# UbiquityRobotics/fiducials

Measured on AMD Instinct MI355X. Metric: frames/sec @1920x1080 20-marker (aruco detect + pose hot path), higher is better.
Workload: dtype u8

## Files before the change

fiducials_amd/csrc/fid_kernels.hip:

```cpp
#include <hip/hip_runtime.h>
#include <stdint.h>
#include <float.h>
#include <limits.h>

#include <type_traits>
#include <utility>

#include "fid_device.h"
#include "../../include/fid_abi.h"

#define WAVE 64

__device__ __forceinline__ int lane_id() { return threadIdx.x & (WAVE - 1); }

__device__ __forceinline__ unsigned long long ballot64(int pred) { return __ballot(pred); }

#define FID_DPP(OLD, V, CTRL, RMASK) __builtin_amdgcn_update_dpp((OLD), (V), (CTRL), (RMASK), 0xf, false)
#define FID_DPP_SCAN_STEPS(STEP) STEP(0x111, 0xf) STEP(0x112, 0xf) STEP(0x114, 0xf) STEP(0x118, 0xf) STEP(0x142, 0xa) STEP(0x143, 0xc)

__device__ __forceinline__ int wave_iscan(int v)
{
#define S_(C, M) v += FID_DPP(0, v, C, M);
    FID_DPP_SCAN_STEPS(S_)
#undef S_
    return v;
}

__device__ __forceinline__ unsigned long long wave_max_u64(unsigned long long k)
{
    unsigned lo = (unsigned)k, hi = (unsigned)(k >> 32);
#define S_(C, M)                                                                      \
    {                                                                                 \
        const unsigned ol = (unsigned)FID_DPP(0, (int)lo, C, M), oh = (unsigned)FID_DPP(0, (int)hi, C, M); \
        const bool gt = oh > hi || (oh == hi && ol > lo);                             \
        lo = gt ? ol : lo;                                                            \
        hi = gt ? oh : hi;                                                            \
    }
    FID_DPP_SCAN_STEPS(S_)
#undef S_
    lo = (unsigned)__builtin_amdgcn_readlane((int)lo, 63);
    hi = (unsigned)__builtin_amdgcn_readlane((int)hi, 63);
    return ((unsigned long long)hi << 32) | lo;
}

__device__ __forceinline__ void wave_argmax_first(unsigned d, unsigned idx, unsigned &md, unsigned &mi)
{
    unsigned v = d;
#define S_(C, M)                                                  \
    {                                                             \
        const unsigned o = (unsigned)FID_DPP(0, (int)v, C, M);    \
        v = o > v ? o : v;                                        \
    }
    FID_DPP_SCAN_STEPS(S_)
#undef S_
    md = (unsigned)__builtin_amdgcn_readlane((int)v, 63);
    unsigned w = d == md ? idx : 0xffffffffu;
#define S_(C, M)                                                  \
    {                                                             \
        const unsigned o = (unsigned)FID_DPP(-1, (int)w, C, M);   \
        w = o < w ? o : w;                                        \
    }
    FID_DPP_SCAN_STEPS(S_)
#undef S_
    mi = (unsigned)__builtin_amdgcn_readlane((int)w, 63);
}

__device__ __forceinline__ double wave_max_nonneg_f64(double v)
{
    unsigned long long u = __double_as_longlong(v);
    unsigned lo = (unsigned)u, hi = (unsigned)(u >> 32);
#define S_(C, M)                                                                                           \
    {                                                                                                      \
        const unsigned ol = (unsigned)FID_DPP(0, (int)lo, C, M), oh = (unsigned)FID_DPP(0, (int)hi, C, M); \
        const bool gt = oh > hi || (oh == hi && ol > lo);  \
        lo = gt ? ol : lo;                                                                                 \
        hi = gt ? oh : hi;                                                                                 \
    }
    FID_DPP_SCAN_STEPS(S_)
#undef S_
    lo = (unsigned)__builtin_amdgcn_readlane((int)lo, 63);
    hi = (unsigned)__builtin_amdgcn_readlane((int)hi, 63);
    return __longlong_as_double(((unsigned long long)hi << 32) | lo);
}

__device__ __forceinline__ int wave_min_i32(int v)
{
#define S_(C, M)                                  \
    {                                             \
        const int o = FID_DPP(INT_MAX, v, C, M);  \
        v = o < v ? o : v;                        \
    }
    FID_DPP_SCAN_STEPS(S_)
#undef S_
    return __builtin_amdgcn_readlane(v, 63);
}
__device__ __forceinline__ int wave_min_i32_dpp(int v) { return wave_min_i32(v); }

__device__ __forceinline__ int wave_sum_i32(int v) { return __builtin_amdgcn_readlane(wave_iscan(v), 63); }

__device__ __forceinline__ long long wave_sum_i64(long long v)
{
    unsigned lo = (unsigned)v, hi = (unsigned)((unsigned long long)v >> 32);
#define S_(C, M)                                                                      \
    {                                                                                 \
        const unsigned ol = (unsigned)FID_DPP(0, (int)lo, C, M), oh = (unsigned)FID_DPP(0, (int)hi, C, M); \
        const unsigned long long t = (((unsigned long long)hi << 32) | lo) + (((unsigned long long)oh << 32) | ol); \
        lo = (unsigned)t;                                                             \
        hi = (unsigned)(t >> 32);                                                     \
    }
    FID_DPP_SCAN_STEPS(S_)
#undef S_
    lo = (unsigned)__builtin_amdgcn_readlane((int)lo, 63);
    hi = (unsigned)__builtin_amdgcn_readlane((int)hi, 63);
    return (long long)(((unsigned long long)hi << 32) | lo);
}

__device__ __forceinline__ double bcast_f64(double v, int src)
{
    const unsigned long long u = __double_as_longlong(v);
    const int l = __builtin_amdgcn_readfirstlane(src);
    const unsigned lo = (unsigned)__builtin_amdgcn_readlane((int)(unsigned)u, l);
    const unsigned hi = (unsigned)__builtin_amdgcn_readlane((int)(unsigned)(u >> 32), l);
    return __longlong_as_double(((unsigned long long)hi << 32) | lo);
}

__device__ __forceinline__ double shfl_f64(double v, int src)
{
    unsigned long long u = __double_as_longlong(v);
    unsigned lo = __shfl((unsigned)u, src, WAVE);
    unsigned hi = __shfl((unsigned)(u >> 32), src, WAVE);
    return __longlong_as_double(((unsigned long long)hi << 32) | lo);
}

__global__ __launch_bounds__(256) void k_to_gray(const uint8_t *__restrict__ src, int stride, long long fstride,
                                                  int enc, uint8_t *__restrict__ dst, int W, int H, int F)
{
    long long total = (long long)W * H * F;
    for (long long i = (long long)blockIdx.x * blockDim.x + threadIdx.x; i < total; i += (long long)gridDim.x * blockDim.x) {
        int x = (int)(i % W);
        long long t = i / W;
        int y = (int)(t % H);
        int f = (int)(t / H);
        const uint8_t *s = src + f * fstride + (long long)y * stride;
        uint8_t v;
        if (enc == FID_ENC_MONO8) {
            v = s[x];
        } else {
            const int px = (enc == FID_ENC_BGRA8 || enc == FID_ENC_RGBA8) ? 4 : 3;
            int c0 = s[px * x], c1 = s[px * x + 1], c2 = s[px * x + 2];
            const bool bfirst = enc == FID_ENC_BGR8 || enc == FID_ENC_BGRA8;
            int b = bfirst ? c0 : c2, r = bfirst ? c2 : c0;
            v = (uint8_t)((b * 3735 + c1 * 19235 + r * 9798 + (1 << 14)) >> 15);
        }
        dst[i] = v;
    }
}

__device__ __forceinline__ int k0_gray(int b, int g, int r) { return (b * 3735 + g * 19235 + r * 9798 + (1 << 14)) >> 15; }
__device__ __forceinline__ int k0_scale16(const uint8_t *p, bool be)
{
    const unsigned v = be ? ((unsigned)p[0] << 8) | p[1] : (unsigned)p[0] | ((unsigned)p[1] << 8);
    const float a = (float)(255. / 65535.);
    const int r = __float2int_rn((float)v * a);
    return r < 0 ? 0 : (r > 255 ? 255 : r);
}
__device__ __forceinline__ int k0_sat8(int v) { return v < 0 ? 0 : (v > 255 ? 255 : v); }
__device__ __forceinline__ int k0_bayer_gray(const int n[9], bool is_green, int hv)
{
    int own, other, green;
    if (is_green) {
        green = n[4];
        other = (n[1] + n[7] + 1) >> 1;
        own = (n[3] + n[5] + 1) >> 1;
    } else {
        own = n[4];
        green = (n[1] + n[3] + n[5] + n[7] + 2) >> 2;
        other = (n[0] + n[2] + n[6] + n[8] + 2) >> 2;
    }
    const int b = hv > 0 ? other : own, r = hv > 0 ? own : other;
    return k0_gray(b, green, r);
}
__global__ __launch_bounds__(256) void k_raw_to_gray(const uint8_t *__restrict__ src, int stride, long long fstride, int enc,
                                                      uint8_t *__restrict__ dst, int W, int H)
{
    const int x0 = ((int)blockIdx.x * 64 + (int)threadIdx.x) * 4, y = (int)blockIdx.y * 4 + (int)threadIdx.y, f = blockIdx.z;
    if (x0 >= W || y >= H) return;
    const uint8_t *img = src + (long long)f * fstride;
    uint8_t *o = dst + ((long long)f * H + y) * W + x0;
    const int n = W - x0 < 4 ? W - x0 : 4;
    const int base = enc & 0xff;
    const bool be = (enc & FID_ENC_BIGENDIAN) != 0;
    int g[4] = {0, 0, 0, 0};
    if (base >= FID_ENC_BAYER_RGGB8 && base <= FID_ENC_BAYER_GRBG8) {
        const int blue0 = (base == FID_ENC_BAYER_RGGB8 || base == FID_ENC_BAYER_GRBG8) ? -1 : 1;
        const int green0 = (base == FID_ENC_BAYER_GBRG8 || base == FID_ENC_BAYER_GRBG8) ? 1 : 0;
        const int yy = y < 1 ? 1 : (y > H - 2 ? H - 2 : y);
        const int hv = ((yy - 1) & 1) ? -blue0 : blue0;
        const int gs = green0 ^ ((yy - 1) & 1);
        const uint8_t *r0 = img + (long long)(yy - 1) * stride, *r1 = r0 + stride, *r2 = r1 + stride;
        if (x0 >= 1 && x0 + 4 <= W - 1) {
            int a0[6], a1[6], a2[6];
#pragma unroll
            for (int k = 0; k < 6; k++) {
                a0[k] = r0[x0 - 1 + k];
                a1[k] = r1[x0 - 1 + k];
                a2[k] = r2[x0 - 1 + k];
            }
#pragma unroll
            for (int k = 0; k < 4; k++) {
                const int nb[9] = {a0[k], a0[k + 1], a0[k + 2], a1[k], a1[k + 1], a1[k + 2], a2[k], a2[k + 1], a2[k + 2]};
                g[k] = k0_bayer_gray(nb, (gs ^ ((x0 + k - 1) & 1)) != 0, hv);
            }
        } else {
            for (int k = 0; k < n; k++) {
                const int x = x0 + k, xx = x < 1 ? 1 : (x > W - 2 ? W - 2 : x);
                const int nb[9] = {r0[xx - 1], r0[xx], r0[xx + 1], r1[xx - 1], r1[xx], r1[xx + 1], r2[xx - 1], r2[xx], r2[xx + 1]};
                g[k] = k0_bayer_gray(nb, (gs ^ ((xx - 1) & 1)) != 0, hv);
            }
        }
    } else if (base == FID_ENC_MONO16) {
        const uint8_t *s = img + (long long)y * stride + 2 * x0;
        for (int k = 0; k < n; k++) g[k] = k0_scale16(s + 2 * k, be);
    } else if (base >= FID_ENC_BGR16 && base <= FID_ENC_RGBA16) {
        const int ch = (base == FID_ENC_BGRA16 || base == FID_ENC_RGBA16) ? 4 : 3;
        const bool bfirst = base == FID_ENC_BGR16 || base == FID_ENC_BGRA16;
        const uint8_t *s = img + (long long)y * stride + 2 * ch * x0;
        for (int k = 0; k < n; k++) {
            const int c0 = k0_scale16(s + 2 * (ch * k), be), c1 = k0_scale16(s + 2 * (ch * k + 1), be), c2 = k0_scale16(s + 2 * (ch * k + 2), be);
            g[k] = k0_gray(bfirst ? c0 : c2, c1, bfirst ? c2 : c0);
        }
    } else {
        const int CY = 1220542, CUB = 2116026, CUG = -409993, CVG = -852492, CVR = 1673527, SH = 20;
        const uint8_t *s = img + (long long)y * stride + 2 * x0;
        for (int k = 0; k < n; k += 2) {
            const int u = s[2 * k] - 128, y0 = s[2 * k + 1], v = s[2 * k + 2] - 128, y1 = s[2 * k + 3];
            const int ruv = (1 << (SH - 1)) + CVR * v, guv = (1 << (SH - 1)) + CVG * v + CUG * u, buv = (1 << (SH - 1)) + CUB * u;
            const int p0 = (y0 - 16 > 0 ? y0 - 16 : 0) * CY, p1 = (y1 - 16 > 0 ? y1 - 16 : 0) * CY;
            g[k] = k0_gray(k0_sat8((p0 + buv) >> SH), k0_sat8((p0 + guv) >> SH), k0_sat8((p0 + ruv) >> SH));
            g[k + 1] = k0_gray(k0_sat8((p1 + buv) >> SH), k0_sat8((p1 + guv) >> SH), k0_sat8((p1 + ruv) >> SH));
        }
    }
    if (n == 4 && (((unsigned long long)o) & 3ull) == 0) {
        *reinterpret_cast<unsigned *>(o) = (unsigned)g[0] | ((unsigned)g[1] << 8) | ((unsigned)g[2] << 16) | ((unsigned)g[3] << 24);
    } else {
        for (int k = 0; k < n; k++) o[k] = (uint8_t)g[k];
    }
}

template <int TX, int TY, int NT>
__global__ __launch_bounds__(NT) void k_threshold(const uint8_t *__restrict__ gray, long long gfstride,
                                                   uint32_t *__restrict__ masks, const DevParams P)
{
    extern __shared__ uint32_t I[];
    const int R = P.rmax;
    const int RW = TX + 2 * R, RH = TY + 2 * R;
    const int PT = (RW + 1) | 1;
    const int tid = threadIdx.x, lane = tid & 63, wid = tid >> 6;
    constexpr int NWAVES = NT / 64;
    const int x0 = blockIdx.x * TX, y0 = blockIdx.y * TY, f = blockIdx.z;
    const uint8_t *g = gray + (long long)f * gfstride;
    const int W = P.W, H = P.H, gs = P.gstride;

    for (int i = tid; i < PT; i += NT) I[i] = 0;
    for (int i = tid; i <= RH; i += NT) I[i * PT] = 0;
    for (int ry = wid; ry < RH; ry += NWAVES) {
        int gy = y0 - R + ry;
        gy = gy < 0 ? 0 : (gy >= H ? H - 1 : gy);
        const uint8_t *grow = g + (long long)gy * gs;
        int carry = 0;
        for (int c = 0; c < RW; c += 64) {
            int rx = c + lane;
            int gx = x0 - R + rx;
            gx = gx < 0 ? 0 : (gx >= W ? W - 1 : gx);
            int v = rx < RW ? (int)grow[gx] : 0;
            v = wave_iscan(v) + carry;
            if (rx < RW) I[(ry + 1) * PT + rx + 1] = (uint32_t)v;
            carry = __shfl(v, 63, WAVE);
        }
    }
    __syncthreads();
    for (int cx = 1 + tid; cx <= RW; cx += NT) {
        uint32_t acc = 0;
#pragma unroll 4
        for (int ry = 1; ry <= RH; ry++) {
            acc += I[ry * PT + cx];
            I[ry * PT + cx] = acc;
        }
    }
    __syncthreads();
    constexpr int SEGS = TX / 64;
    const int S = P.nscales, TC = P.TC;
    const long long plane = (long long)P.TR * TC * MT_ROWS;
    for (int item = wid; item < TY * SEGS; item += NWAVES) {
        int ty = item / SEGS, seg = item % SEGS;
        int x = seg * 64 + lane;
        int gx = x0 + x, gy = y0 + ty;
        if (gy >= H) continue;
        int valid = gx < W;
        int gv = valid ? (int)g[(long long)gy * gs + gx] : 0;
        int t2 = 2 * (gv + P.idelta) - 1;
        int rc = ty + R, cc = x + R;
        uint32_t *mrow = masks + (long long)f * S * plane + mask_word(TC, gy + 1, MASK_PADW + ((x0 + seg * 64) >> 5));
        for (int s = 0; s < S; s++) {
            int win = P.win[s], r = win >> 1;
            const uint32_t *top = I + (rc - r) * PT, *bot = I + (rc + r + 1) * PT;
            int sum = (int)(bot[cc + r + 1] - top[cc + r + 1] - bot[cc - r] + top[cc - r]);
            int fg = valid && (2 * sum >= t2 * win * win);
            unsigned long long b = ballot64(fg);
            if (lane == 0) {
                mrow[(long long)s * plane] = (uint32_t)b;
                mrow[(long long)s * plane + MT_ROWS] = (uint32_t)(b >> 32);
            }
        }
    }
}

template <int NT, int WT>
__global__ __launch_bounds__(NT) void k_threshold_wide(const uint8_t *__restrict__ gray, long long gfstride,
                                                        uint32_t *__restrict__ masks, const DevParams P, int BH)
{
    extern __shared__ unsigned long long HP[];
    constexpr int NWAVES = NT / 64;
    const int tid = threadIdx.x, lane = tid & 63, wid = tid >> 6;
    const int W = P.W, H = P.H, gs = P.gstride, S = P.nscales, TC = P.TC;
    const int f = blockIdx.z, y0 = blockIdx.x * BH;
    if (y0 >= H) return;
    const int y1 = y0 + BH < H ? y0 + BH : H;
    const uint8_t *g = gray + (long long)f * gfstride;
    const long long plane = (long long)P.TR * TC * MT_ROWS;
    uint32_t *mframe = masks + (long long)f * S * plane;
    unsigned long long *wtot = HP + W + 1;
    const int K = (W + NT - 1) / NT;
    const int c0 = tid * K;
    const int nk = c0 >= W ? 0 : (W - c0 < K ? W - c0 : K);
    const int nseg = (W + 63) / 64;
    for (int s = 0; s < S; s++) {
        const int win = P.win[s], r = win >> 1;
        const long long area = (long long)win * win;
        uint32_t V[WT];
        {
            const int lo = y0 - r > 0 ? y0 - r : 0, hi = y0 + r < H - 1 ? y0 + r : H - 1;
            const uint32_t nabove = r > y0 ? (uint32_t)(r - y0) : 0u, nbelow = y0 + r > H - 1 ? (uint32_t)(y0 + r - (H - 1)) : 0u;
#pragma unroll
            for (int j = 0; j < WT; j++) V[j] = 0;
            for (int yy = lo; yy <= hi; yy++) {
                const uint8_t *row = g + (long long)yy * gs + c0;
#pragma unroll
                for (int j = 0; j < WT; j++)
                    if (j < nk) V[j] += row[j];
            }
            const uint8_t *top = g + c0, *bot = g + (long long)(H - 1) * gs + c0;
#pragma unroll
            for (int j = 0; j < WT; j++)
                if (j < nk) V[j] += nabove * top[j] + nbelow * bot[j];
        }
        for (int y = y0; y < y1; y++) {
            if (y > y0) {
                const int yin = y + r < H - 1 ? y + r : H - 1, yout = y - 1 - r > 0 ? y - 1 - r : 0;
                const uint8_t *ri = g + (long long)yin * gs + c0, *ro = g + (long long)yout * gs + c0;
#pragma unroll
                for (int j = 0; j < WT; j++)
                    if (j < nk) V[j] += (uint32_t)ri[j] - (uint32_t)ro[j];
            }
            unsigned long long tot = 0;
#pragma unroll
            for (int j = 0; j < WT; j++)
                if (j < nk) tot += V[j];
// ... 1932 lines not shown
                }
            }
        }
        {
            const bool had = state == ST_ACTIVE;
            const bool mv = had || state == ST_NEED;
            int nbr = br, nbc = bc;
            if (mv) {
                const int xb = cx + (MASK_PADW * 32 - 1), yy = cy;
                const int sdx = cx - cxp, sdy = cy - cyp;
                if (had) {
                    nbr = sdy >= 2 ? (yy >> 4) : sdy <= -2 ? ((yy + 2) >> 4) - 1 : br;
                    nbc = sdx >= 2 ? (xb >> 5) : sdx <= -2 ? ((xb + 2) >> 5) - 1 : bc;
                } else {
                    nbr = sdy > 0 ? (yy >> 4) : sdy < 0 ? ((yy + 2) >> 4) - 1 : ((yy & 15) >= 8 ? (yy >> 4) : (yy >> 4) - 1);
                    nbc = sdx > 0 ? (xb >> 5) : sdx < 0 ? ((xb + 2) >> 5) - 1 : ((xb & 31) >= 16 ? (xb >> 5) : (xb >> 5) - 1);
                }
                nbr = nbr < 0 ? 0 : (nbr > TR - 2 ? TR - 2 : nbr);
                nbc = nbc < 0 ? 0 : (nbc > TC - 2 ? TC - 2 : nbc);
                cxp = cx;
                cyp = cy;
            }
            const bool moved = mv && (!had || nbr != br || nbc != bc);
            if (ballot64(moved)) {
                static_for<4>([&](auto sc) {
                    constexpr int s = decltype(sc)::value, pr = s >> 1, pcx = s & 1;
                    const int ntr = nbr + ((pr ^ nbr) & 1), ntc = nbc + ((pcx ^ nbc) & 1);
                    const int otr = br + ((pr ^ br) & 1), otc = bc + ((pcx ^ bc) & 1);
                    if (moved && (!had || ntr != otr || ntc != otc)) {
                        const uint32_t *g = pl + ((long long)ntr * TC + ntc) * MT_ROWS;
                        static_for<4>([&](auto qc) {
                            constexpr int q = decltype(qc)::value;
                            __builtin_amdgcn_global_load_lds((const __attribute__((address_space(1))) void *)g,
                                                             (__attribute__((address_space(3))) void *)((char *)s_win + (pcx * 8 + pr * 4 + q) * 1024 - q * 16),
                                                             16, q * 16, 0);
                        });
                    }
                });
                if (moved) {
                    pend = 1;
                    pbr = nbr;
                    pbc = nbc;
                    if (had) {
                        const int r0 = nbr > br ? nbr : br, c0 = nbc > bc ? nbc : bc;
                        vyb = r0 * MT_ROWS;
                        vys = (unsigned)((nbr == br ? 2 : 1) * MT_ROWS - 3);
                        vxb = c0 * 32;
                        vxs = (unsigned)((nbc == bc ? 2 : 1) * 32 - 3);
                        const unsigned xr = (unsigned)(cx + (MASK_PADW * 32 - 1) - vxb), rr = (unsigned)(cy - vyb);
                        if (xr > vxs || rr > vys) state = ST_LOADING;
                    } else {
                        state = ST_LOADING;
                    }
                }
            }
        }
#ifdef FID_DEBUG_STATS
        d_ckcyc += __builtin_readcyclecounter() - d_c0;
#endif
        if (all_done && ballot64(state != ST_IDLE) == 0) break;
        const int work_left = !all_done;
        for (int it = 0; it < SW_RUN; it++) {
            const unsigned long long act = ballot64(state == ST_ACTIVE);
            if (it >= SW_CKPT && ballot64(state != ST_ACTIVE && (state != ST_IDLE || work_left))) break;
            if (act == 0) break;
#ifdef FID_DEBUG_STATS
            d_iters++;
            d_active += __popcll(act);
#endif
            if (state == ST_ACTIVE) {
                const unsigned raw = raw_here();
                const unsigned e = s_lut[raw | ((unsigned)sdir << 8)];
                const unsigned skey = seed_key(cx, cy, sdir);
                const bool onseed = ((e & 0x20u) && (cx & sgm) == 0) || ((e & 0x40u) && (cy & sgm) == 0);
                if (count > 0 && onseed) {
                    state = ST_FINAL;
                } else if (count > 0 && skey == brkey) {
                    ok = 0;
                    state = ST_FINAL;
                } else {
                    if ((count & (count - 1)) == 0) brkey = skey;
                    {
                        const bool lo = (e & 8u) && (unsigned)pc < ko, lh = (e & 16u) && (unsigned)pc + 1u < kh;
                        ko = lo ? (unsigned)pc : ko;
                        po = lo ? (unsigned)count : po;
                        kh = lh ? (unsigned)pc + 1u : kh;
                        ph = lh ? (unsigned)count : ph;
                    }
                    const int sn = e & 7;
                    acc = __builtin_amdgcn_alignbit((uint32_t)sn, acc, 4);
                    if ((count & 7) == 7) pool[((count & CK ? chunkB : chunkA) * CKW) + (unsigned)((count & (CK - 1)) >> 3)] = acc;
                    count++;
                    const int dx = dir_dx(sn), dy = dir_dy(sn);
                    cx += dx;
                    cy += dy;
                    pc += __mul24(dy, W2) + dx;
                    sdir = sn ^ 4;
                    const unsigned xr = (unsigned)(cx + (MASK_PADW * 32 - 1) - vxb), rr = (unsigned)(cy - vyb);
                    state = (xr > vxs || rr > vys) ? ST_NEED : ST_ACTIVE;
                }
            }
        }
    }
    if (ovf) atomicOr(&G->overflow, ovf);
#ifdef FID_DEBUG_STATS
    if (lane == 0) {
        atomicAdd(&G->dbg[0], d_iters);
        atomicAdd(&G->dbg[1], d_ckpts);
        atomicAdd(&G->dbg[2], d_active);
        atomicAdd(&G->dbg[3], d_ckcyc);
        atomicAdd(&G->dbg[6], (unsigned long long)(__builtin_readcyclecounter() - d_t0));
        atomicAdd(&G->dbg[7], 1ull);
        for (int k = 0; k < 4; k++) atomicAdd(&G->dbg[21 + k], d_lanes[k]);
    }
#endif
}

__global__ __launch_bounds__(256) void k_seg_link2(const uint2 *__restrict__ seedq, DevSegC *__restrict__ segs,
                                                    const unsigned long long *__restrict__ seedhash, const DevCounts *__restrict__ counts,
                                                    const DevParams P)
{
    const int f = blockIdx.y;
    unsigned ns = (unsigned)counts[f].nseeds;
    ns = ns < (unsigned)P.maxContours ? ns : (unsigned)P.maxContours;
    const unsigned long long *fsh = seedhash + (long long)f * P.seedHashCap;
    const uint2 *fsq = seedq + (long long)f * P.maxContours;
    DevSegC *fsg = segs + (long long)f * P.maxContours;
    for (unsigned i = blockIdx.x * blockDim.x + threadIdx.x; i < ns; i += gridDim.x * blockDim.x) {
        if (fsg[i].n == SEG_INVALID) continue;
        const unsigned nx = seedhash_find(fsh, P.seedHashCap, P.seedGen, seedhash_key(fsg[i].next_key, (int)(fsq[i].x >> 27)));
        if (nx < ns) {
            fsg[i].next_idx = nx;
            fsg[nx].linked = 1u;
        }
    }
}

template <unsigned SC_HOPS>
__global__ __launch_bounds__(64) void k_seg_cycles(const uint2 *__restrict__ seedq, const DevSegC *__restrict__ segs,
                                                    const DevPend *__restrict__ pend, const uint4 *__restrict__ wres,
                                                    uint4 *__restrict__ contours, uint4 *__restrict__ cinfo, uint32_t *__restrict__ cbase,
                                                    uint4 *__restrict__ recs, DevCounts *__restrict__ counts, DevGlobal *__restrict__ G,
                                                    const DevParams P, int part, int warm)
{
    __shared__ uint2 s_hops[SC_HOPS ? SC_HOPS : 1][SC_HOPS ? 64 : 1];
    const int f = blockIdx.y;
    const int lane = lane_id();
    unsigned ns = (unsigned)counts[f].nseeds, nv = (unsigned)counts[f].nsurv;
    ns = ns < (unsigned)P.maxContours ? ns : (unsigned)P.maxContours;
    nv = nv < (unsigned)P.maxContours ? nv : (unsigned)P.maxContours;
    const unsigned lcap = (unsigned)P.maxContours / 2u, rcap = (unsigned)P.maxContours;
    const uint2 *fsq = seedq + (long long)f * P.maxContours;
    const DevSegC *fsg = segs + (long long)f * P.maxContours;
    const DevPend *fpd = pend + (long long)f * P.maxContours;
    uint4 *fco = contours + (long long)f * P.maxContours + (part ? lcap : 0u);
    uint4 *fci = cinfo + (long long)f * P.maxContours + (part ? lcap : 0u);
    uint32_t *fcb = cbase + (long long)f * P.maxContours + (part ? lcap : 0u);
    uint4 *frc = recs + (long long)f * 2 * P.maxContours + (part ? rcap : 0u);
    unsigned *cnt_slots = (unsigned *)(part ? &counts[f].ncontours2 : &counts[f].ncontours);
    unsigned *cnt_recs = (unsigned *)(part ? &counts[f].nrec2 : &counts[f].nrec);
    const unsigned dcap = (unsigned)P.maxChunks * CK;
    const unsigned W2 = (unsigned)P.W + 2u;
    const unsigned ibeg = part ? ns : 0u, iend = part ? ns + nv : ns;
    if (warm && !part) {
        const unsigned nlines = (ns * (unsigned)sizeof(DevSegC) + 127u) >> 7, nx = (gridDim.x + 7u) >> 3;
        unsigned acc = 0;
        for (unsigned k = (blockIdx.x >> 3) * 64u + (unsigned)lane; k < nlines; k += nx * 64u)
            acc += *reinterpret_cast<const volatile uint32_t *>(reinterpret_cast<const char *>(fsg) + (size_t)k * 128u);
        asm volatile("" ::"v"(acc));
    }
    for (unsigned i0 = ibeg + blockIdx.x * 64; i0 < iend; i0 += gridDim.x * 64) {
        const unsigned i = i0 + lane;
        int accept = 0, hole = 0;
        unsigned L = 0, key = 0, hops = 0, pos = 0, n0 = 0, nx0 = SEG_INVALID;
        uint2 st = make_uint2(0u, 0u);
        if (i < ns) {
            const DevSegC s = fsg[i];
            if (s.n != SEG_INVALID && s.n != 0u && s.linked && (s.ko & s.kh) != 0xffffffffu) {
                bool co = s.ko != 0xffffffffu, ch = s.kh != 0xffffffffu, closed = false;
                unsigned KO = s.ko, KH = s.kh, cur = s.next_idx;
                L = s.n;
                hops = 1;
                while (cur != SEG_INVALID) {
                    if (cur == i) {
                        closed = true;
                        break;
                    }
                    DevSegC r;
                    {
                        const uint4 q = reinterpret_cast<const uint4 *>(fsg + cur)[0];
                        r.next_idx = q.x;
                        r.n = q.y;
                        r.ko = q.z;
                        r.kh = q.w;
                    }
                    if (r.n == SEG_INVALID || r.n == 0u) break;
                    co = co && !(r.ko < s.ko);
                    ch = ch && !(r.kh < s.kh);
                    if (!co && !ch) break;
                    KO = r.ko < KO ? r.ko : KO;
                    KH = r.kh < KH ? r.kh : KH;
                    L += r.n;
                    if (SC_HOPS && hops - 1u < SC_HOPS) s_hops[hops - 1u][lane] = make_uint2(cur, r.n);
                    hops++;
                    if (L > (unsigned)P.maxPerim) break;
                    cur = r.next_idx;
                }
                if (closed && L >= (unsigned)P.minPerim && L <= (unsigned)P.maxPerim) {
                    if (co && KO < KH) {
                        accept = 1;
                        hole = 0;
                        key = s.ko;
                        pos = s.pos & 0xffffu;
                    } else if (ch && KH < KO) {
                        accept = 1;
                        hole = 1;
                        key = s.kh;
                        pos = s.pos >> 16;
                    }
                }
                if (accept) {
                    n0 = s.n;
                    nx0 = s.next_idx;
                    const unsigned ky = key / W2, kx = key - ky * W2;
                    st = make_uint2((kx - 1u - (unsigned)hole) | ((ky - 1u) << 16), (uint32_t)f | ((fsq[i].x >> 27) << 16) | ((uint32_t)hole << 24));
                }
            }
        } else if (i < iend) {
            const unsigned j = i - ns;
            if (!fpd[j].p) {
                const uint4 w = wres[(long long)f * P.maxContours + j];
                if (w.z) {
                    st = make_uint2(w.x, w.y);
                    L = w.z;
                    key = w.w;
                    accept = 2;
                }
            }
        }
        const unsigned long long mk = ballot64(accept);
        if (mk) {
            const unsigned myL = accept ? (L + 7u) & ~7u : 0u, myR = accept == 1 ? hops + 1u : (accept == 2 ? 1u : 0u);
            const unsigned sL = wave_iscan_dpp(myL), sR = wave_iscan_dpp(myR);
            const unsigned totL = (unsigned)__builtin_amdgcn_readlane((int)sL, 63), totR = (unsigned)__builtin_amdgcn_readlane((int)sR, 63);
            unsigned bslot = 0, bdense = 0, brec = 0;
            if (lane == 63) {
                bslot = atomicAdd(cnt_slots, (unsigned)__popcll(mk));
                bdense = atomicAdd((unsigned *)&counts[f].ndense, totL);
                brec = atomicAdd(cnt_recs, totR);
            }
            bslot = (unsigned)__builtin_amdgcn_readlane((int)bslot, 63);
            bdense = (unsigned)__builtin_amdgcn_readlane((int)bdense, 63);
            brec = (unsigned)__builtin_amdgcn_readlane((int)brec, 63);
            const unsigned idx = bslot + (unsigned)__popcll(mk & ((1ull << lane) - 1ull));
            if (accept) {
                if (idx < lcap) {
                    fco[idx] = make_uint4(st.x, st.y, L, key);
                    fci[idx] = make_uint4(i, pos, nx0, 0u);
                    const unsigned dst0 = bdense + sL - myL;
                    unsigned rec = brec + sR - myR;
                    if (dst0 + L > dcap || rec + myR > rcap) {
                        atomicOr(&G->overflow, 8u);
                        fcb[idx] = SEG_INVALID;
                    } else if (accept == 2) {
                        fcb[idx] = dst0;
                        frc[rec] = make_uint4((unsigned)P.maxContours + (i - ns), dst0, L, REC_NO_CHUNK);
                    } else {
                        fcb[idx] = dst0;
                        const unsigned ck0 = fsg[i].chunk0;
                        frc[rec++] = make_uint4(i, dst0, (n0 - pos) | (pos << 16), ck0);
                        unsigned off = n0 - pos, cur = nx0;
                        {
                            const unsigned noted = !SC_HOPS ? 0u : (hops - 1u < SC_HOPS ? hops - 1u : SC_HOPS);
                            for (unsigned h = 0; h < noted; h++) {
                                const uint2 e = s_hops[h][lane];
                                frc[rec++] = make_uint4(e.x, dst0 + off, e.y, fsg[e.x].chunk0);
                                off += e.y;
                                cur = e.x;
                            }
                            if (noted) cur = hops - 1u > noted ? fsg[cur].next_idx : i;
                        }
                        while (cur != i && cur != SEG_INVALID && off < L) {
                            const uint2 q = reinterpret_cast<const uint2 *>(fsg + cur)[0];
                            frc[rec++] = make_uint4(cur, dst0 + off, q.y, fsg[cur].chunk0);
                            off += q.y;
                            cur = q.x;
                        }
                        frc[rec++] = make_uint4(i, dst0 + off, pos, ck0);
                        for (; rec < brec + sR; rec++) frc[rec] = make_uint4(0u, 0u, 0u, 0u);
                    }
                } else {
                    atomicOr(&G->overflow, 2u);
                }
            }
        }
    }
}

#define K4_SHORT_PTS 2048
#define K4_SHORT_STACK 256
#define K4_LONG_STACK 1024
__device__ __host__ inline int pts_cap_first(const DevParams &P) { return P.maxPerim < K4_SHORT_PTS ? P.maxPerim : K4_SHORT_PTS; }

#define K4_RETRY_BIT (1u << 25)
__global__ __launch_bounds__(64) void k_approx(uint4 *__restrict__ contours, const uint32_t *__restrict__ chunk_tab,
                                                const uint32_t *__restrict__ pool, DevCand *__restrict__ cands,
                                                DevCounts *__restrict__ counts, DevGlobal *__restrict__ G, const DevParams P,
                                                int pts_cap, int stack_cap, int second_pass, const uint32_t *__restrict__ dense,
                                                const uint32_t *__restrict__ cbase, int part = 0)
{
    extern __shared__ __attribute__((aligned(16))) uint32_t pts[];
    int2 *stack = reinterpret_cast<int2 *>(pts + pts_cap);
    __shared__ int dst[2 * 16];
    const int lane = lane_id();
    const int f = blockIdx.y;
    unsigned n = (unsigned)(dense ? (part == 2 ? counts[f].ncontours2 : counts[f].ncontours) : counts[f].nsurv);
    n = n < (unsigned)P.maxStarts ? n : (unsigned)P.maxStarts;
    n = n < (unsigned)P.maxContours ? n : (unsigned)P.maxContours;
    const unsigned loff = part == 2 ? (unsigned)P.maxContours / 2u : 0u;
    if (part) n = n < (unsigned)P.maxContours / 2u ? n : (unsigned)P.maxContours / 2u;
    const int W = P.W, H = P.H;
    uint4 *fco = contours + (long long)f * P.maxContours + loff;
    const uint32_t *fpool = pool;
    for (unsigned cb = blockIdx.x; cb < n; cb += gridDim.x * 64) {
      const unsigned myci = cb + (unsigned)lane * gridDim.x;
      uint4 mine = make_uint4(0u, 0u, 0u, 0u);
      if (myci < n) mine = fco[myci];
      int take = mine.z != 0;
      if (second_pass) take = take && ((int)mine.z > pts_cap_first(P) || (mine.y & K4_RETRY_BIT));
      else take = take && (int)mine.z <= pts_cap;
      unsigned long long todo = ballot64(take);
      while (todo) {
        const int src = __ffsll((long long)todo) - 1;
        todo &= todo - 1;
        const unsigned ci = cb + (unsigned)src * gridDim.x;
        uint4 c;
        c.x = (unsigned)__builtin_amdgcn_readlane((int)mine.x, src);
        c.y = (unsigned)__builtin_amdgcn_readlane((int)mine.y, src);
        c.z = (unsigned)__builtin_amdgcn_readlane((int)mine.z, src);
        c.w = (unsigned)__builtin_amdgcn_readlane((int)mine.w, src);
        const int count = (int)c.z;
        const int x0 = c.x & 0xffff, y0 = c.x >> 16;
        const int s = (c.y >> 16) & 0xff, hole = (c.y >> 24) & 1;
        __syncthreads();
        uint32_t pref = 0x80000000u | ci;
        if (dense) {
            const uint32_t cb0 = cbase[(long long)f * P.maxContours + loff + ci];
            if (cb0 == SEG_INVALID) continue;
            pref = cb0;
            const uint8_t *src = reinterpret_cast<const uint8_t *>(dense) + (long long)f * P.maxChunks * CK + cb0;
            uint32_t base = c.x;
            for (int k0 = 0; k0 < count; k0 += 512) {
                const int k = k0 + 8 * lane;
                uint2 w = make_uint2(0u, 0u);
                if (k < count) w = *reinterpret_cast<const uint2 *>(src + k);
                base = codes8_to_points(pts, k, count, base, w);
            }
        } else {
            uint32_t base = c.x;
            for (int k0 = 0; k0 < count; k0 += 512) {
                const int k = k0 + 8 * lane;
                uint32_t w = 0u;
                if (k < count)
                    w = fpool[(long long)chunk_tab[chunk_tab_at(P, f, (unsigned)P.maxContours + ci, (unsigned)k >> 6)] * CKW + ((k & (CK - 1)) >> 3)];
                base = codes8_to_points(pts, k, count, base, codes_nibbles_to_bytes(w));
            }
        }
        __syncthreads();
        double eps = (double)count * P.polyAcc;
        eps *= eps;
        int new_count = 0, reject = 0, top = 0;
        int rs_start = 0, pos = 0, le_eps = 0;
        int sx = 0, sy = 0;
        for (int it = 0; it < 3; it++) {
            pos = (pos + rs_start) % count;
            uint32_t sp = pts[pos];
            sx = sp & 0xffff;
            sy = sp >> 16;
            unsigned bd = 0, bj = 0;
            for (int j = 1 + lane; j < count; j += 64) {
                int idx = pos + j;
                idx = idx >= count ? idx - count : idx;
                uint32_t p = pts[idx];
                int dx = (int)(p & 0xffff) - sx, dy = (int)(p >> 16) - sy;
                unsigned d = (unsigned)(dx * dx + dy * dy);
                const bool gt = d > bd;
                bd = gt ? d : bd;
                bj = gt ? (unsigned)j : bj;
            }
            unsigned md, mj;
            wave_argmax_first(bd, bd ? bj : 0xffffffffu, md, mj);
            if (md > 0) rs_start = (int)mj;
            le_eps = (double)md <= eps;
        }
        if (!le_eps) {
            int2 rs, sl;
            rs.y = sl.x = pos % count;
            sl.y = rs.x = (rs_start + sl.x) % count;
            if (lane == 0) {
                stack[0] = rs;
                stack[1] = sl;
            }
            top = 2;
        } else {
            if (lane == 0) {
                dst[0] = sx;
                dst[1] = sy;
            }
            new_count = 1;
        }
        __syncthreads();
        while (top > 0 && !reject) {
            int2 sl = stack[--top];
            uint32_t ep = pts[sl.y];
            int ex = ep & 0xffff, ey = ep >> 16;
            uint32_t sp = pts[sl.x];
            sx = sp & 0xffff;
            sy = sp >> 16;
            int mcount = sl.y - sl.x;
            if (mcount < 0) mcount += count;
            mcount -= 1;
            int split = 0;
            if (mcount > 0) {
                int dx = ex - sx, dy = ey - sy;
                unsigned lbd = 0, lbt = 0;
                bool any = false;
                for (int t = lane; t < mcount; t += 64) {
                    int idx = sl.x + 1 + t;
                    idx = idx >= count ? idx - count : idx;
                    uint32_t p = pts[idx];
                    int px = p & 0xffff, py = p >> 16;
                    int cr = (py - sy) * dx - (px - sx) * dy;
                    unsigned d = (unsigned)(cr < 0 ? -cr : cr);
                    const bool gt = d > lbd || !any;
                    lbd = gt ? d : lbd;
                    lbt = gt ? (unsigned)t : lbt;
                    any = true;
                }
                unsigned mdist, mt;
                wave_argmax_first(any ? lbd : 0u, any ? lbt : 0xffffffffu, mdist, mt);
                double max_dist = (double)mdist;
                int bt = (int)mt;
                le_eps = max_dist * max_dist <= eps * ((double)dx * dx + (double)dy * dy);
                if (!le_eps) {
                    split = sl.x + 1 + bt;
                    split = split >= count ? split - count : split;
                }
            } else {
                le_eps = 1;
            }
            __syncthreads();
            if (le_eps) {
                if (new_count >= 9) {
                    reject = 1;
                } else {
                    if (lane == 0) {
                        dst[2 * new_count] = sx;
                        dst[2 * new_count + 1] = sy;
                    }
                    new_count++;
                }
            } else {
                if (top + 2 > stack_cap) {
                    reject = 1;
                    if (lane == 0) {
                        if (second_pass) atomicOr(&G->overflow, 4u);
                        else fco[ci].y = c.y | K4_RETRY_BIT;
                    }
                } else {
                    if (lane == 0) {
                        stack[top] = make_int2(split, sl.y);
                        stack[top + 1] = make_int2(sl.x, split);
                    }
                    top += 2;
                }
            }
            __syncthreads();
        }
        if (reject || new_count < 4) continue;
        {
            const int cnt = new_count;
            int posd = cnt - 1, wpos, i;
            int spx, spy, ptx, pty, epx, epy;
#define RD(X, Y)                  \
    do {                          \
        X = dst[2 * posd];        \
        Y = dst[2 * posd + 1];    \
        if (++posd >= cnt) posd = 0; \
    } while (0)
            RD(spx, spy);
            wpos = posd;
            RD(ptx, pty);
            for (i = 0; i < cnt && new_count > 2; i++) {
                RD(epx, epy);
                double dx = epx - spx, dy = epy - spy;
                double dist = fabs((double)(ptx - spx) * dy - (double)(pty - spy) * dx);
                double sip = (double)(ptx - spx) * (epx - ptx) + (double)(pty - spy) * (epy - pty);
                __syncthreads();
                if (dist * dist <= 0.5 * eps * (dx * dx + dy * dy) && dx != 0 && dy != 0 && sip >= 0) {
                    new_count--;
                    spx = epx;
                    spy = epy;
                    if (lane == 0) {
                        dst[2 * wpos] = spx;
                        dst[2 * wpos + 1] = spy;
                    }
                    if (++wpos >= cnt) wpos = 0;
                    __syncthreads();
                    RD(ptx, pty);
                    i++;
                    continue;
                }
                spx = ptx;
                spy = pty;
                if (lane == 0) {
                    dst[2 * wpos] = spx;
                    dst[2 * wpos + 1] = spy;
                }
                if (++wpos >= cnt) wpos = 0;
                ptx = epx;
                pty = epy;
                __syncthreads();
            }
#undef RD
        }
        __syncthreads();
        if (new_count != 4) continue;
        int ax[4], ay[4];
#pragma unroll
        for (int k = 0; k < 4; k++) {
            ax[k] = dst[2 * k];
            ay[k] = dst[2 * k + 1];
        }
        {
            int prevx = ax[2], prevy = ay[2], curx = ax[3], cury = ay[3];
            int dx0 = curx - prevx, dy0 = cury - prevy, orientation = 0, convex = 1;
#pragma unroll
            for (int k = 0; k < 4; k++) {
                prevx = curx;
                prevy = cury;
                curx = ax[k];
                cury = ay[k];
                int dx = curx - prevx, dy = cury - prevy;
                int dxdy0 = dx * dy0, dydx0 = dy * dx0;
                orientation |= (dydx0 > dxdy0) ? 1 : ((dydx0 < dxdy0) ? 2 : 3);
                if (orientation == 3) convex = 0;
                dx0 = dx;
                dy0 = dy;
            }
            if (!convex) continue;
        }
        {
            int maxdim = W > H ? W : H;
            double minDistSq = (double)maxdim * maxdim;
#pragma unroll
            for (int k = 0; k < 4; k++) {
                int k1 = (k + 1) & 3;
                double d = (double)(ax[k] - ax[k1]) * (double)(ax[k] - ax[k1]) + (double)(ay[k] - ay[k1]) * (double)(ay[k] - ay[k1]);
                minDistSq = minDistSq < d ? minDistSq : d;
            }
            double mcd = (double)count * P.minCornerDistRate;
            if (minDistSq < mcd * mcd) continue;
            int tooNear = 0;
#pragma unroll
            for (int k = 0; k < 4; k++)
                if (ax[k] < P.minDistToBorder || ay[k] < P.minDistToBorder || ax[k] > W - 1 - P.minDistToBorder ||
                    ay[k] > H - 1 - P.minDistToBorder)
                    tooNear = 1;
            if (tooNear) continue;
        }
        if (lane == 0) {
            int o = atomicAdd(&counts[f].ncand, 1);
            if (o < P.maxCands) {
                DevCand cd;
                cd.scale = s;
                cd.size = count;
                cd.sx = x0;
                cd.sy = y0;
                cd.hole = hole;
                cd.key = c.w;
                cd.pref = pref;
                cd.pad = 0;
#pragma unroll
                for (int k = 0; k < 4; k++) {
                    cd.c[2 * k] = (float)ax[k];
                    cd.c[2 * k + 1] = (float)ay[k];
                }
                cands[(long long)f * P.maxCands + o] = cd;
            } else {
                atomicOr(&counts[f].overflow, 1);
            }
        }
      }
    }
}

__global__ __launch_bounds__(256) void k_sort_cands(const DevCand *__restrict__ cands, DevCand *__restrict__ sorted,
                                                    float4 *__restrict__ cmeta, DevCounts *__restrict__ counts, const DevParams P)
{
    extern __shared__ unsigned long long keys[];
    __shared__ int s_rank[256];
    const int f = blockIdx.x;
    int n = counts[f].ncand;
    n = n < P.maxCands ? n : P.maxCands;
    if ((int)blockIdx.y * (gridDim.y > 1 ? 64 : 256) >= n) return;
    const DevCand *src = cands + (long long)f * P.maxCands;
    DevCand *dstc = sorted + (long long)f * P.maxCands;
    for (int i = threadIdx.x; i < n; i += blockDim.x)
        keys[i] = ((unsigned long long)(unsigned)src[i].scale << 32) | (0xffffffffu - src[i].key);
    __syncthreads();
    const int parts = gridDim.y > 1 ? 4 : 1, ipb = 256 / parts;
    const int il = threadIdx.x & (ipb - 1), part = threadIdx.x / ipb;
    const int j0 = (int)((long long)n * part / parts), j1 = (int)((long long)n * (part + 1) / parts);
    for (int i0 = (int)blockIdx.y * ipb; i0 < n; i0 += (int)gridDim.y * ipb) {
        const int i = i0 + il;
        if (part == 0) s_rank[il] = 0;
        __syncthreads();
        DevCand c;
        if (i < n) {
            if (part == 0) c = src[i];
            const unsigned long long k = keys[i];
            int r = 0;
            for (int j = j0; j < j1; j++) r += keys[j] < k;
            atomicAdd(&s_rank[il], r);
        }
        __syncthreads();
        if (i < n && part == 0) {
            const int rank = s_rank[il];
            double dx1 = c.c[2] - c.c[0], dy1 = c.c[3] - c.c[1];
            double dx2 = c.c[4] - c.c[0], dy2 = c.c[5] - c.c[1];
            double cross = (dx1 * dy2) - (dy1 * dx2);
            if (cross < 0.0) {
                float tx = c.c[2], ty = c.c[3];
                c.c[2] = c.c[6];
                c.c[3] = c.c[7];
                c.c[6] = tx;
                c.c[7] = ty;
            }
            dstc[rank] = c;
            cmeta[(long long)f * P.maxCands + rank] =
                make_float4(c.c[0] + c.c[2] + c.c[4] + c.c[6], c.c[1] + c.c[3] + c.c[5] + c.c[7], (float)c.size, 0.f);
        }
        __syncthreads();
    }
}

__device__ __forceinline__ int near_row_off(int i, int nw)
{
    const int q = i >> 5;
    return i * nw - 16 * q * (q - 1) - (i - 32 * q) * q;
}
__global__ __launch_bounds__(256) void k_near(const DevCand *__restrict__ sorted, const float4 *__restrict__ cmeta,
                                               uint32_t *__restrict__ nearb, const DevCounts *__restrict__ counts,
                                               const DevParams P)
{
    const int f = blockIdx.y;
    int n = counts[f].ncand;
    n = n < P.maxCands ? n : P.maxCands;
    const int NW = P.maxCands >> 5;
    const int nw = (n + 31) >> 5, nw2 = (n + 63) >> 6;
    const DevCand *cs = sorted + (long long)f * P.maxCands;
    const float4 *cm = cmeta + (long long)f * P.maxCands;
    uint32_t *nb = nearb + (long long)f * P.maxCands * NW;
    const int lane = lane_id();
    const float rate_f = (float)P.minMarkerDistRate * 1.0001f;
    const int wave = (int)(blockIdx.x * (blockDim.x >> 6) + (threadIdx.x >> 6)), nwaves = (int)(gridDim.x * (blockDim.x >> 6));
    auto item = [&](int i, int w2) {
        const int j = w2 * 64 + lane;
        const bool valid = j > i && j < n;
        const float4 ma = cm[i];
        bool close = false;
        if (valid) {
            const float4 mo = cm[j];
            const float sz = ma.z < mo.z ? ma.z : mo.z;
            const float lim0 = sz * rate_f;
            const float lim = 16.f * (lim0 * lim0 * 1.001f + 1.f) + 1.f;
            const float dx = ma.x - mo.x, dy = ma.y - mo.y;
            close = dx * dx + dy * dy < lim;
        }
        bool near = false;
        if (close) {
            const DevCand a = cs[i];
            const DevCand o = cs[j];
            const int minimumPerimeter = a.size < o.size ? a.size : o.size;
            double mmd = (double)minimumPerimeter * P.minMarkerDistRate;
            mmd = mmd * mmd;
#pragma unroll
            for (int fc = 0; fc < 4; fc++) {
                double distSq = 0;
#pragma unroll
                for (int c = 0; c < 4; c++) {
                    const int modC = (c + fc) & 3;
                    const float ax = a.c[2 * modC] - o.c[2 * c];
                    const float ay = a.c[2 * modC + 1] - o.c[2 * c + 1];
                    distSq += ax * ax + ay * ay;
                }
                distSq /= 4.;
                near = near || distSq < mmd;
            }
        }
        const unsigned long long bits = ballot64(near);
        if (lane < 2) {
            const int w = 2 * w2 + lane;
            if (w >= (i >> 5) && w < nw) nb[near_row_off(i, nw) + w - (i >> 5)] = (uint32_t)(bits >> (32 * lane));
        }
    };
    if (nwaves <= n) {
        __shared__ uint32_t s_row[4][128];
        __shared__ uint16_t s_q[4][128];
        const int wv = (int)(threadIdx.x >> 6);
        uint32_t *row = s_row[wv];
        uint16_t *q = s_q[wv];
        row[lane] = 0u;
        row[lane + 64] = 0u;
        for (int i = __builtin_amdgcn_readfirstlane(wave); i < n; i += nwaves) {
            const float4 ma = cm[i];
            const DevCand a = cs[i];
            int qn = 0;
            auto exact = [&](int cnt) {
                bool near = false;
                int j = 0;
                if (lane < cnt) {
                    j = q[lane];
                    const DevCand o = cs[j];
                    const int minimumPerimeter = a.size < o.size ? a.size : o.size;
                    double mmd = (double)minimumPerimeter * P.minMarkerDistRate;
                    mmd = mmd * mmd;
#pragma unroll
                    for (int fc = 0; fc < 4; fc++) {
                        double distSq = 0;
#pragma unroll
                        for (int c = 0; c < 4; c++) {
                            const int modC = (c + fc) & 3;
                            const float ax = a.c[2 * modC] - o.c[2 * c];
                            const float ay = a.c[2 * modC + 1] - o.c[2 * c + 1];
                            distSq += ax * ax + ay * ay;
                        }
                        distSq /= 4.;
                        near = near || distSq < mmd;
                    }
                }
                if (near) atomicOr(&row[j >> 5], 1u << (j & 31));
            };
            for (int w2 = i >> 6; w2 < nw2; w2++) {
                const int j = w2 * 64 + lane;
                bool close = false;
                if (j > i && j < n) {
                    const float4 mo = cm[j];
                    const float sz = ma.z < mo.z ? ma.z : mo.z;
                    const float lim0 = sz * rate_f;
                    const float lim = 16.f * (lim0 * lim0 * 1.001f + 1.f) + 1.f;
                    const float dx = ma.x - mo.x, dy = ma.y - mo.y;
                    close = dx * dx + dy * dy < lim;
                }
                const unsigned long long cb = ballot64(close);
                if (cb) {
                    if (close) q[qn + __popcll(cb & ((1ull << lane) - 1ull))] = (uint16_t)j;
                    qn += __popcll(cb);
                    if (qn >= 64) {
                        exact(64);
                        qn -= 64;
                        if (lane < qn) {
                            const uint16_t t = q[64 + lane];
                            q[lane] = t;
                        }
                    }
                }
            }
            if (qn) exact(qn);
            for (int w = (i >> 5) + lane; w < nw; w += 64) {
                nb[near_row_off(i, nw) + w - (i >> 5)] = row[w];
                row[w] = 0u;
            }
        }
    } else {
        for (int it = wave; it < n * nw2; it += nwaves) {
            const int i = it / nw2, w2 = it - i * nw2;
            if (w2 * 64 + 63 < i) continue;
            item(i, w2);
        }
    }
}

__global__ __launch_bounds__(1024) void k_resolve(const DevCand *__restrict__ sorted, const uint32_t *__restrict__ nearb,
                                                 DevCand *__restrict__ filtered, DevCounts *__restrict__ counts,
                                                 unsigned *__restrict__ worklist, unsigned *__restrict__ nwork,
                                                 const DevParams P, int lds_words, DevGlobal *__restrict__ G, int reg_max)
{
#ifdef FID_DEBUG_STATS
    unsigned long long d_t[8];
    int d_k = 0, d_iters = 0;
#define RES_MARK() d_t[d_k++] = __builtin_readcyclecounter();
#else
#define RES_MARK()
#endif
    RES_MARK()
    extern __shared__ int sizes[];
    __shared__ uint32_t s_rem[128];
    __shared__ uint32_t s_alive[128];
    __shared__ int s_off[128];
    __shared__ int s_mem[16][64];
    const int f = blockIdx.x, lane = lane_id(), tid = threadIdx.x, nt = blockDim.x;
    int n = counts[f].ncand;
    n = n < P.maxCands ? n : P.maxCands;
    const int NW = P.maxCands >> 5;
    const DevCand *cs = sorted + (long long)f * P.maxCands;
    const uint32_t *nb = nearb + (long long)f * P.maxCands * NW;
    const int nw = (n + 31) >> 5;
    int *label = sizes + P.maxCands, *csize = label + P.maxCands;
    uint32_t *s_near = reinterpret_cast<uint32_t *>(csize + P.maxCands);
    const int tri = n > 0 ? near_row_off(n - 1, nw) + nw - ((n - 1) >> 5) : 0;
    const bool in_lds = tri <= lds_words;
    for (int i = tid; i < n; i += nt) {
        sizes[i] = cs[i].size;
        label[i] = i;
        csize[i] = 0;
    }
    if (tid < 128) s_rem[tid] = 0u;
    if (in_lds) {
        const uint4 *src = reinterpret_cast<const uint4 *>(nb);
        uint4 *dst = reinterpret_cast<uint4 *>(s_near);
        const int nq = (tri + 3) >> 2;
        for (int t0 = 0; t0 < nq; t0 += 4 * nt) {
            uint4 v[4];
#pragma unroll
            for (int u = 0; u < 4; u++) {
                const int t = t0 + u * nt + tid;
                v[u] = t < nq ? src[t] : make_uint4(0u, 0u, 0u, 0u);
            }
#pragma unroll
            for (int u = 0; u < 4; u++) {
                const int t = t0 + u * nt + tid;
                if (t < nq) dst[t] = v[u];
            }
        }
    }
// ... 1763 lines not shown
```

Measured before the change: 37250.

## Rework k_approx Douglas-Peucker: packed argmax keys, register vertex list, fewer barriers

Factors the farthest-point searches in the polygon approximation kernel into a templated helper. For contours of up to 2046 points it packs distance and inverted index into one 32-bit key, reduced with a single DPP max, and uses packed 16-bit subtract plus sdot2 for the distance math. The output vertex list moves from shared memory into a per-lane register read back with readlane, which removes several __syncthreads. The recursion stack keeps the current segment in registers so only one segment is pushed per split. The risk is key overflow if distances exceed 21 bits, and subtle changes to tie-break and traversal order.

```diff
diff --git a/fiducials_amd/csrc/fid_kernels.hip b/fiducials_amd/csrc/fid_kernels.hip
--- a/fiducials_amd/csrc/fid_kernels.hip
+++ b/fiducials_amd/csrc/fid_kernels.hip
@@ -63,6 +63,18 @@
     FID_DPP_SCAN_STEPS(S_)
 #undef S_
     mi = (unsigned)__builtin_amdgcn_readlane((int)w, 63);
+}
+
+__device__ __forceinline__ unsigned wave_max_u32(unsigned v)
+{
+#define S_(C, M)                                                  \
+    {                                                             \
+        const unsigned o = (unsigned)FID_DPP(0, (int)v, C, M);    \
+        v = o > v ? o : v;                                        \
+    }
+    FID_DPP_SCAN_STEPS(S_)
+#undef S_
+    return (unsigned)__builtin_amdgcn_readlane((int)v, 63);
 }
 
 __device__ __forceinline__ double wave_max_nonneg_f64(double v)
@@ -2601,6 +2613,70 @@
 #define K4_LONG_STACK 1024
 __device__ __host__ inline int pts_cap_first(const DevParams &P) { return P.maxPerim < K4_SHORT_PTS ? P.maxPerim : K4_SHORT_PTS; }
 
+#define K4_KEY_PTS 2046
+#define K4_KEY_IDX_BITS 11
+#define K4_KEY_IDX_MASK ((1u << K4_KEY_IDX_BITS) - 1u)
+
+template <bool KEY, bool SLICE>
+__device__ __forceinline__ void approx_farthest(const uint32_t *pts, int lane, int count, int base, int first, int n_end, int sx, int sy,
+                                                int dx, int dy, unsigned &md, unsigned &mi)
+{
+    const unsigned wrap = 4u * (unsigned)count;
+    unsigned off = 4u * (unsigned)(base + first + lane);
+    off = min(off, off - wrap);
+    const char *const pb = reinterpret_cast<const char *>(pts);
+    const uint32_t spk = (uint32_t)sx | ((uint32_t)sy << 16);
+    const thr_s16x2 nrm = {(short)-dy, (short)dx};
+    unsigned bd = 0, bn = 0, key = 0;
+    bool any = false;
+#define APPROX_DIST_(D)                                          \
+    const uint32_t p = *reinterpret_cast<const uint32_t *>(pb + off); \
+    off += 256u;                                                 \
+    off = min(off, off - wrap);                                  \
+    unsigned D;                                                  \
+    if constexpr (KEY) {                                         \
+         \
+        const thr_s16x2 q = __builtin_bit_cast(thr_s16x2, pk_sub16(p, spk)); \
+        const int cr = __builtin_amdgcn_sdot2(q, SLICE ? nrm : q, 0, false); \
+        D = (unsigned)(SLICE && cr < 0 ? -cr : cr);              \
+    } else {                                                     \
+        const int px = p & 0xffff, py = p >> 16;                 \
+        if constexpr (SLICE) {                                   \
+            const int cr = (py - sy) * dx - (px - sx) * dy;      \
+            D = (unsigned)(cr < 0 ? -cr : cr);                   \
+        } else {                                                 \
+            const int ex = px - sx, ey = py - sy;                \
+            D = (unsigned)(ex * ex + ey * ey);                   \
+        }                                                        \
+    }
+    if constexpr (KEY) {
+        const int kn_end = (int)K4_KEY_IDX_MASK - n_end;
+        for (int kn = (int)K4_KEY_IDX_MASK - (first + lane); kn > kn_end; kn -= 64) {
+            APPROX_DIST_(d)
+            const unsigned k = (d << K4_KEY_IDX_BITS) | (unsigned)kn;
+            key = k > key ? k : key;
+        }
+    } else {
+        for (int n = first + lane; n < n_end; n += 64) {
+            APPROX_DIST_(d)
+            const bool gt = SLICE ? (d > bd || !any) : d > bd;
+            bd = gt ? d : bd;
+            bn = gt ? (unsigned)n : bn;
+            any = true;
+        }
+    }
+#undef APPROX_DIST_
+    if constexpr (KEY) {
+        const unsigned m = wave_max_u32(key);
+        md = m >> K4_KEY_IDX_BITS;
+        mi = K4_KEY_IDX_MASK - (m & K4_KEY_IDX_MASK);
+    } else if constexpr (SLICE) {
+        wave_argmax_first(any ? bd : 0u, any ? bn : 0xffffffffu, md, mi);
+    } else {
+        wave_argmax_first(bd, bd ? bn : 0xffffffffu, md, mi);
+    }
+}
+
 #define K4_RETRY_BIT (1u << 25)
 __global__ __launch_bounds__(64) void k_approx(uint4 *__restrict__ contours, const uint32_t *__restrict__ chunk_tab,
                                                 const uint32_t *__restrict__ pool, DevCand *__restrict__ cands,
@@ -2610,7 +2686,6 @@
 {
     extern __shared__ __attribute__((aligned(16))) uint32_t pts[];
     int2 *stack = reinterpret_cast<int2 *>(pts + pts_cap);
-    __shared__ int dst[2 * 16];
     const int lane = lane_id();
     const int f = blockIdx.y;
     unsigned n = (unsigned)(dense ? (part == 2 ? counts[f].ncontours2 : counts[f].ncontours) : counts[f].nsurv);
@@ -2666,54 +2741,58 @@
             }
         }
         __syncthreads();
+        const bool keyed = count <= K4_KEY_PTS;
         double eps = (double)count * P.polyAcc;
         eps *= eps;
         int new_count = 0, reject = 0, top = 0;
         int rs_start = 0, pos = 0, le_eps = 0;
         int sx = 0, sy = 0;
+        uint32_t dstv = 0;
+#define DST_PUT(K, XY) dstv = lane == (K) ? (uint32_t)(XY) : dstv
+#define DST_GET(K) ((uint32_t)__builtin_amdgcn_readlane((int)dstv, (K)))
+        uint32_t sp = 0;
         for (int it = 0; it < 3; it++) {
-            pos = (pos + rs_start) % count;
-            uint32_t sp = pts[pos];
+            pos += rs_start;
+            pos = pos >= count ? pos - count : pos;
+            sp = (uint32_t)__builtin_amdgcn_readfirstlane((int)pts[pos]);
             sx = sp & 0xffff;
             sy = sp >> 16;
-            unsigned bd = 0, bj = 0;
-            for (int j = 1 + lane; j < count; j += 64) {
-                int idx = pos + j;
-                idx = idx >= count ? idx - count : idx;
-                uint32_t p = pts[idx];
-                int dx = (int)(p & 0xffff) - sx, dy = (int)(p >> 16) - sy;
-                unsigned d = (unsigned)(dx * dx + dy * dy);
-                const bool gt = d > bd;
-                bd = gt ? d : bd;
-                bj = gt ? (unsigned)j : bj;
-            }
             unsigned md, mj;
-            wave_argmax_first(bd, bd ? bj : 0xffffffffu, md, mj);
+            if (keyed) approx_farthest<true, false>(pts, lane, count, pos, 1, count, sx, sy, 0, 0, md, mj);
+            else approx_farthest<false, false>(pts, lane, count, pos, 1, count, sx, sy, 0, 0, md, mj);
             if (md > 0) rs_start = (int)mj;
             le_eps = (double)md <= eps;
         }
+        int2 cur = make_int2(0, 0);
+        int have = 0;
         if (!le_eps) {
-            int2 rs, sl;
-            rs.y = sl.x = pos % count;
-            sl.y = rs.x = (rs_start + sl.x) % count;
-            if (lane == 0) {
-                stack[0] = rs;
-                stack[1] = sl;
-            }
-            top = 2;
+            int far = rs_start + pos;
+            far = far >= count ? far - count : far;
+            if (lane == 0) stack[0] = make_int2(far, pos);
+            cur = make_int2(pos, far);
+            have = 1;
+            top = 1;
         } else {
-            if (lane == 0) {
-                dst[0] = sx;
-                dst[1] = sy;
-            }
+            DST_PUT(0, sp);
             new_count = 1;
         }
         __syncthreads();
-        while (top > 0 && !reject) {
-            int2 sl = stack[--top];
-            uint32_t ep = pts[sl.y];
+        while ((have || top > 0) && !reject) {
+            int2 sl;
+            uint32_t ep;
+            if (have) {
+                sl = cur;
+                have = 0;
+                ep = (uint32_t)__builtin_amdgcn_readfirstlane((int)pts[sl.y]);
+            } else {
+                sl = stack[--top];
+                sl.x = __builtin_amdgcn_readfirstlane(sl.x);
+                sl.y = __builtin_amdgcn_readfirstlane(sl.y);
+                const uint32_t vs = pts[sl.x], ve = pts[sl.y];
+                sp = (uint32_t)__builtin_amdgcn_readfirstlane((int)vs);
+                ep = (uint32_t)__builtin_amdgcn_readfirstlane((int)ve);
+            }
             int ex = ep & 0xffff, ey = ep >> 16;
-            uint32_t sp = pts[sl.x];
             sx = sp & 0xffff;
             sy = sp >> 16;
             int mcount = sl.y - sl.x;
@@ -2722,22 +2801,9 @@
             int split = 0;
             if (mcount > 0) {
                 int dx = ex - sx, dy = ey - sy;
-                unsigned lbd = 0, lbt = 0;
-                bool any = false;
-                for (int t = lane; t < mcount; t += 64) {
-                    int idx = sl.x + 1 + t;
-                    idx = idx >= count ? idx - count : idx;
-                    uint32_t p = pts[idx];
-                    int px = p & 0xffff, py = p >> 16;
-                    int cr = (py - sy) * dx - (px - sx) * dy;
-                    unsigned d = (unsigned)(cr < 0 ? -cr : cr);
-                    const bool gt = d > lbd || !any;
-                    lbd = gt ? d : lbd;
-                    lbt = gt ? (unsigned)t : lbt;
-                    any = true;
-                }
                 unsigned mdist, mt;
-                wave_argmax_first(any ? lbd : 0u, any ? lbt : 0xffffffffu, mdist, mt);
+                if (keyed) approx_farthest<true, true>(pts, lane, count, sl.x + 1, 0, mcount, sx, sy, dx, dy, mdist, mt);
+                else approx_farthest<false, true>(pts, lane, count, sl.x + 1, 0, mcount, sx, sy, dx, dy, mdist, mt);
                 double max_dist = (double)mdist;
                 int bt = (int)mt;
                 le_eps = max_dist * max_dist <= eps * ((double)dx * dx + (double)dy * dy);
@@ -2753,10 +2819,7 @@
                 if (new_count >= 9) {
                     reject = 1;
                 } else {
-                    if (lane == 0) {
-                        dst[2 * new_count] = sx;
-                        dst[2 * new_count + 1] = sy;
-                    }
+                    DST_PUT(new_count, sp);
                     new_count++;
                 }
             } else {
@@ -2767,11 +2830,10 @@
                         else fco[ci].y = c.y | K4_RETRY_BIT;
                     }
                 } else {
-                    if (lane == 0) {
-                        stack[top] = make_int2(split, sl.y);
-                        stack[top + 1] = make_int2(sl.x, split);
-                    }
-                    top += 2;
+                    if (lane == 0) stack[top] = make_int2(split, sl.y);
+                    top += 1;
+                    cur = make_int2(sl.x, split);
+                    have = 1;
                 }
             }
             __syncthreads();
@@ -2781,11 +2843,12 @@
             const int cnt = new_count;
             int posd = cnt - 1, wpos, i;
             int spx, spy, ptx, pty, epx, epy;
-#define RD(X, Y)                  \
-    do {                          \
-        X = dst[2 * posd];        \
-        Y = dst[2 * posd + 1];    \
-        if (++posd >= cnt) posd = 0; \
+#define RD(X, Y)                         \
+    do {                                 \
+        const uint32_t q_ = DST_GET(posd); \
+        X = q_ & 0xffff;                 \
+        Y = q_ >> 16;                    \
+        if (++posd >= cnt) posd = 0;     \
     } while (0)
             RD(spx, spy);
             wpos = posd;
@@ -2795,42 +2858,35 @@
                 double dx = epx - spx, dy = epy - spy;
                 double dist = fabs((double)(ptx - spx) * dy - (double)(pty - spy) * dx);
                 double sip = (double)(ptx - spx) * (epx - ptx) + (double)(pty - spy) * (epy - pty);
-                __syncthreads();
                 if (dist * dist <= 0.5 * eps * (dx * dx + dy * dy) && dx != 0 && dy != 0 && sip >= 0) {
                     new_count--;
                     spx = epx;
                     spy = epy;
-                    if (lane == 0) {
-                        dst[2 * wpos] = spx;
-                        dst[2 * wpos + 1] = spy;
-                    }
+                    DST_PUT(wpos, (uint32_t)spx | ((uint32_t)spy << 16));
                     if (++wpos >= cnt) wpos = 0;
-                    __syncthreads();
                     RD(ptx, pty);
                     i++;
                     continue;
                 }
                 spx = ptx;
                 spy = pty;
-                if (lane == 0) {
-                    dst[2 * wpos] = spx;
-                    dst[2 * wpos + 1] = spy;
-                }
+                DST_PUT(wpos, (uint32_t)spx | ((uint32_t)spy << 16));
                 if (++wpos >= cnt) wpos = 0;
                 ptx = epx;
                 pty = epy;
-                __syncthreads();
             }
 #undef RD
         }
-        __syncthreads();
         if (new_count != 4) continue;
         int ax[4], ay[4];
 #pragma unroll
         for (int k = 0; k < 4; k++) {
-            ax[k] = dst[2 * k];
-            ay[k] = dst[2 * k + 1];
-        }
+            const uint32_t q = DST_GET(k);
+            ax[k] = q & 0xffff;
+            ay[k] = q >> 16;
+        }
+#undef DST_PUT
+#undef DST_GET
         {
             int prevx = ax[2], prevy = ay[2], curx = ax[3], cury = ay[3];
             int dx0 = curx - prevx, dy0 = cury - prevy, orientation = 0, convex = 1;
```

Result: faster. 37760, median of 6 (+1.4%).
